# ksil/LFPSQP.jl

Hardware: AMD Instinct MI355X
Metric: projected-CG iters/sec at n=1e7, m=128 fp64 (higher is better)
Workload: dtype f64

## Files before the change

lfpsqp.jl_amd/csrc/context.hip:

```cpp
#include <dlfcn.h>
#include <stdarg.h>
#include <stdio.h>
#include <stdlib.h>
#include <ctype.h>
#include <string.h>

#include <algorithm>

#include "internal.h"

namespace lfpsqp {

int set_err(lfpsqp_ctx* ctx, int code, const char* fmt, ...) {
    char buf[1024];
    va_list ap;
    va_start(ap, fmt);
    vsnprintf(buf, sizeof(buf), fmt, ap);
    va_end(ap);
    if (ctx) ctx->err = buf;
    else fprintf(stderr, "lfpsqp: %s\n", buf);
    return code;
}

int ensure_part(lfpsqp_ctx* ctx, size_t doubles) {
// ... 228 lines not shown
}

__global__ __launch_bounds__(lfpsqp::kThreads) void view_copy_kernel(const double* __restrict__ A, const double* __restrict__ rs, const double* __restrict__ u,
                                                                     const double* __restrict__ w, double* __restrict__ D, int64_t ld, int64_t n, int m) {
    const int64_t i = ((int64_t)blockIdx.x * lfpsqp::kThreads + threadIdx.x) * 2;
    if (i >= n) return;
    const double2 s = rs ? lfpsqp::ld2(rs + i) : make_double2(1.0, 1.0);
    const double2 uu = u ? lfpsqp::ld2(u + i) : make_double2(0.0, 0.0);
    const bool v1 = i + 1 < n;
    const int j0 = blockIdx.y * 16, j1 = (j0 + 16 < m) ? j0 + 16 : m;
#pragma unroll 4
    for (int j = j0; j < j1; ++j) {
        const double2 c = lfpsqp::ld2(A + (int64_t)j * ld + i);
        const double wj = u ? w[j] : 0.0;
        const double2 o = make_double2(fma(uu.x, wj, s.x * c.x), fma(uu.y, wj, s.y * c.y));
        if (v1) lfpsqp::st2(D + (int64_t)j * ld + i, o);
        else D[(int64_t)j * ld + i] = o.x;
    }
}

extern "C" {

int lfpsqp_ctx_create(int device, lfpsqp_ctx** out) {
    if (!out) return LFPSQP_ERR_ARG;
    *out = nullptr;
    int ndev = 0;
    if (hipGetDeviceCount(&ndev) != hipSuccess || ndev <= 0) return set_err(nullptr, LFPSQP_ERR_HIP, "no HIP device visible");
    if (device < 0 || device >= ndev) return set_err(nullptr, LFPSQP_ERR_ARG, "device %d out of range (%d visible)", device, ndev);
    lfpsqp_ctx* ctx = new lfpsqp_ctx();
    ctx->device = device;
    if (hipSetDevice(device) != hipSuccess) { delete ctx; return set_err(nullptr, LFPSQP_ERR_HIP, "hipSetDevice(%d) failed", device); }
    hipDeviceProp_t prop;
    if (hipGetDeviceProperties(&prop, device) == hipSuccess) {
        ctx->devname = std::string(prop.name) + " (" + prop.gcnArchName + ")";
        ctx->num_cu = prop.multiProcessorCount;
        ctx->real_gpu = strncmp(prop.gcnArchName, "gfx", 3) == 0;
    }
    bool ok = hipStreamCreate(&ctx->stream) == hipSuccess;
    ok = ok && hipMalloc((void**)&ctx->scal, 64 * sizeof(double)) == hipSuccess;
    ok = ok && hipMalloc((void**)&ctx->istat, 128 * sizeof(int64_t)) == hipSuccess;
    ok = ok && hipHostMalloc((void**)&ctx->h_scal, 4 * 64 * sizeof(double)) == hipSuccess;
    ok = ok && hipHostMalloc((void**)&ctx->h_istat, 4 * 16 * sizeof(int64_t)) == hipSuccess;
    for (int i = 0; ok && i < 4; ++i) ok = hipEventCreate(&ctx->ev_slot[i]) == hipSuccess;
    ok = ok && hipEventCreate(&ctx->ev_t0) == hipSuccess && hipEventCreate(&ctx->ev_t1) == hipSuccess;
    if (ok) ok = hipMemset(ctx->scal, 0, 64 * sizeof(double)) == hipSuccess && hipMemset(ctx->istat, 0, 128 * sizeof(int64_t)) == hipSuccess;
    if (!ok) { delete ctx; return set_err(nullptr, LFPSQP_ERR_HIP, "context resource allocation failed"); }
    if (const char* e = getenv("LFPSQP_ONEPASS")) ctx->tune_onepass = atoi(e);
    if (const char* e = getenv("LFPSQP_SPGRAM")) ctx->tune_spgram = atoi(e) < 0 ? -1 : 0;
    if (const char* e = getenv("LFPSQP_VEC_BLOCKS")) ctx->tune_vec_blocks = atoi(e) > 0 ? atoi(e) : 0;
    if (const char* e = getenv("LFPSQP_NRB_MFMA")) ctx->tune_nrb_mfma = atoi(e) > 0 ? 1 : (atoi(e) < 0 ? -1 : 0);
    if (const char* e = getenv("LFPSQP_GPING")) ctx->tune_gping = atoi(e) == 1 ? 1 : 0;
    if (const char* e = getenv("LFPSQP_NRB_WG_CAP")) ctx->batch_wg_cap = atoi(e) > 0 ? atoi(e) : 0;
    if (const char* e = getenv("LFPSQP_STAGE_ROUNDS")) ctx->stage_cap = atoi(e) > 0 ? atoi(e) : 0;
    *out = ctx;
    return 0;
}

int lfpsqp_ctx_destroy(lfpsqp_ctx* ctx) {
    if (!ctx) return 0;
    (void)hipSetDevice(ctx->device);
    (void)hipStreamSynchronize(ctx->stream);
    if (ctx->comm.kind == Comm::RCCL && ctx->comm.nccl_comm && ctx->comm.ncclCommDestroy) ctx->comm.ncclCommDestroy(ctx->comm.nccl_comm);
    for (int r = 0; r < kP2PMaxRanks; ++r)
        if (ctx->comm.p2p_peer[r] && ctx->comm.p2p_peer[r] != ctx->comm.p2p_mine) (void)hipIpcCloseMemHandle(ctx->comm.p2p_peer[r]);
    if (ctx->comm.p2p_mine) (void)hipFree(ctx->comm.p2p_mine);
    if (ctx->comm.p2p_err) (void)hipHostFree(ctx->comm.p2p_err);
    if (ctx->prof_init)
        for (int s = 0; s < kProfSlots; ++s)
            for (int e = 0; e < kProfEvents; ++e)
                for (int k = 0; k < 2; ++k) (void)hipEventDestroy(ctx->prof_ev[s][e][k]);
    for (int i = 0; i < 4; ++i) if (ctx->ev_slot[i]) (void)hipEventDestroy(ctx->ev_slot[i]);
    if (ctx->ev_t0) (void)hipEventDestroy(ctx->ev_t0);
    if (ctx->ev_t1) (void)hipEventDestroy(ctx->ev_t1);
    if (ctx->part) (void)hipFree(ctx->part);
    if (ctx->small) (void)hipFree(ctx->small);
    if (ctx->d_m) (void)hipFree(ctx->d_m);
    if (ctx->d_qw) (void)hipFree(ctx->d_qw);
    if (ctx->d_zeros) (void)hipFree(ctx->d_zeros);
    if (ctx->d_nvec) (void)hipFree(ctx->d_nvec);
    if (ctx->d_tri) (void)hipFree(ctx->d_tri);
    if (ctx->d_view) (void)hipFree(ctx->d_view);
    if (ctx->h_m) (void)hipHostFree(ctx->h_m);
    if (ctx->scal) (void)hipFree(ctx->scal);
    if (ctx->istat) (void)hipFree(ctx->istat);
    if (ctx->h_scal) (void)hipHostFree(ctx->h_scal);
    if (ctx->h_istat) (void)hipHostFree(ctx->h_istat);
    if (ctx->stream) (void)hipStreamDestroy(ctx->stream);
    delete ctx;
    return 0;
}

int lfpsqp_ctx_sync(lfpsqp_ctx* ctx) {
    LF_ARG(ctx, ctx != nullptr);
    LF_HIP(ctx, hipStreamSynchronize(ctx->stream));
    return 0;
}

const char* lfpsqp_last_error(const lfpsqp_ctx* ctx) { return ctx ? ctx->err.c_str() : "null context"; }

int lfpsqp_device_name(const lfpsqp_ctx* ctx, char* buf, int64_t buflen) {
    if (!ctx || !buf || buflen <= 0) return LFPSQP_ERR_ARG;
    snprintf(buf, (size_t)buflen, "%s", ctx->devname.c_str());
    return 0;
}

int lfpsqp_device_uuid(const lfpsqp_ctx* ctx, char* buf, int64_t buflen) {
// ... 588 lines not shown
```

lfpsqp.jl_amd/csrc/internal.h:

```cpp
#pragma once
#include <hip/hip_runtime.h>
#include <stdint.h>

#include <string>
#include <vector>

#include "../../include/lfpsqp_hip.h"
#include "kernels.h"

struct lfpsqp_slab {
    void* p = nullptr;
    int refs = 0;
};
struct lfpsqp_vec {
    double* p = nullptr;
    int64_t n = 0;
    int64_t cap = 0;
    lfpsqp_slab* slab = nullptr;
};

constexpr int64_t kLdSkewDefault = 16;

struct lfpsqp_mat {
    double* p = nullptr;
// ... 42 lines not shown

    double* part = nullptr;
    size_t part_cap = 0;
    double* small = nullptr;
    size_t small_cap = 0;
    double* d_m = nullptr;
    double* h_m = nullptr;
    size_t m_cap = 0;
    std::vector<double> warm_V;
    int warm_m = 0;
    double* d_view = nullptr;
    double* d_nvec = nullptr;
    size_t nvec_cap = 0;
    double* d_tri = nullptr;
    size_t tri_cap = 0;
    double* d_zeros = nullptr;
    double* d_qw = nullptr;
    size_t qw_cap = 0;
    double* scal = nullptr;
    int64_t* istat = nullptr;
    double* h_scal = nullptr;
    int64_t* h_istat = nullptr;
    hipEvent_t ev_slot[4] = {nullptr, nullptr, nullptr, nullptr};
    hipEvent_t ev_t0 = nullptr, ev_t1 = nullptr;

    int tune_ks = 0;
    bool tune_nt = true;
    int ks_for(int64_t n) const { return tune_ks ? tune_ks : (n >= 4000000 ? 4 : 2); }
    int tune_onepass = 0;
    int tune_spgram = 0;
    int tune_vec_blocks = 0;
    int tune_nrb_mfma = -1;
    int tune_gping = 0;

    bool real_gpu = false;
    int place_tries = 3;
    int64_t place_min_bytes = (int64_t)1 << 30;
    double place_last_ms[64] = {0};
    int place_last_n = 0, place_last_pick = 0;

    struct ProjcgResume {
        bool valid = false;
        const double *x = nullptr, *g = nullptr, *d = nullptr, *Z = nullptr;
        int m = 0;
        int64_t nv = 0, iters = 0;
        bool gcur_is_rp = false;
        const double *dg = nullptr, *b = nullptr;
        double a0 = 0.0;
        int64_t n_global = 0;
        uint64_t epoch = 0;
    } pcg_resume;
    int batch_wg_cap = 0;
    int stage_cap = 0;
    uint64_t launch_epoch = 0;

    bool profiling = false;
    hipEvent_t prof_ev[lfpsqp::kProfSlots][lfpsqp::kProfEvents][2];
    int prof_used[lfpsqp::kProfSlots] = {0};
    int64_t prof_seq[lfpsqp::kProfSlots] = {0};
    bool prof_live[lfpsqp::kProfSlots] = {false};
    int64_t prof_count[lfpsqp::kProfSlots] = {0};
    double prof_ms[lfpsqp::kProfSlots] = {0};
    bool prof_init = false;
};

namespace lfpsqp {

int set_err(lfpsqp_ctx* ctx, int code, const char* fmt, ...);
int ensure_part(lfpsqp_ctx* ctx, size_t doubles);
int ensure_small(lfpsqp_ctx* ctx, size_t doubles);
int ensure_mvec(lfpsqp_ctx* ctx, size_t doubles);
int ensure_nvec(lfpsqp_ctx* ctx, size_t doubles);
int ensure_view(lfpsqp_ctx* ctx);
constexpr int kViewTau = 8;
constexpr int kViewScratch = kViewTau + 4 * 1024 + 64;
int allreduce_dev(lfpsqp_ctx* ctx, double* buf, int64_t count, int op = 0);

void prof_begin(lfpsqp_ctx* ctx, int s);
void prof_end(lfpsqp_ctx* ctx, int s);
void prof_collect(lfpsqp_ctx* ctx);

inline int64_t round_up(int64_t a, int64_t b) { return (a + b - 1) / b * b; }
inline int64_t ntiles_of(int64_t n, int ks) { return (n + (int64_t)kSlabRows * ks - 1) / ((int64_t)kSlabRows * ks); }

#define LF_HIP(ctx, expr)                                                                              \
    do {                                                                                               \
        hipError_t e__ = (expr);                                                                       \
        if (e__ != hipSuccess)                                                                         \
            return lfpsqp::set_err((ctx), LFPSQP_ERR_HIP, "%s failed: %s (%s:%d)", #expr,              \
                                   hipGetErrorString(e__), __FILE__, __LINE__);                        \
    } while (0)

#define LF_TRY(expr)               \
    do {                           \
        int rc__ = (expr);         \
        if (rc__ != 0) return rc__; \
    } while (0)

#define LF_ARG(ctx, cond)                                                                               \
    do {                                                                                                \
        if (!(cond)) return lfpsqp::set_err((ctx), LFPSQP_ERR_ARG, "invalid argument: %s (%s:%d)", #cond, \
                                            __FILE__, __LINE__);                                        \
    } while (0)

#define LF_LAUNCH_CHECK(ctx) LF_HIP(ctx, hipGetLastError())

// ... 355 lines not shown
```

lfpsqp.jl_amd/csrc/projcg.hip:

```cpp
#include <math.h>
#include <stdlib.h>

#include <algorithm>
#include <vector>

#include "internal.h"
#include "sparse.h"
#include "sphess.h"

namespace lfpsqp {

enum { S_DAD = 0, S_RG = 1, S_ALPHA = 2, S_RPGP = 3, S_GPGP = 4, S_BETA = 5, S_NR = 6, S_TOL = 7, S_DD = 8, S_ALPHA_PREV = 9 };
enum { I_STATUS = 0, I_ITER = 1, I_MAXIT = 2 };
enum { ST_RUNNING = 0, ST_CONVERGED = 1, ST_RG_BREAK = 2, ST_NEGCURV = 3, ST_MAXIT = 4 };

struct AOpD {
    double a0;
    const double* dg;
    __device__ __forceinline__ double2 apply(int64_t i, double2 d) const {
        if (dg) {
            const double2 q = ld2(dg + i);
            return make_double2((a0 + q.x) * d.x, (a0 + q.y) * d.y);
        }
        return make_double2(a0 * d.x, a0 * d.y);
    }
};

struct AOpV {
    const double* Av;
    __device__ __forceinline__ double2 apply(int64_t i, double2) const { return ld2(Av + i); }
};

struct AOpLR {
    double a0;
    const double* dg;
    const double* V;
    int64_t ldv;
    int k;
    const double *sigma, *vtv;
    __device__ __forceinline__ double2 apply(int64_t i, double2 d) const {
        double2 o = dg ? make_double2((a0 + dg[i]) * d.x, (a0 + dg[i + 1]) * d.y) : make_double2(a0 * d.x, a0 * d.y);
        for (int j = 0; j < k; ++j) {
            const double c = ld_scal(sigma + j) * ld_scal(vtv + j);
            const double2 v = ld2(V + (int64_t)j * ldv + i);
            o.x = fma(v.x, c, o.x);
            o.y = fma(v.y, c, o.y);
        }
        return o;
    }
};

template <int B>
struct BandD {
    static_assert(B >= 1 && B <= 4, "bandwidth 1 .. 4");
    double a0;
    const double* dg;
    const double* off;
    int64_t ldo;
    int64_t n;
    int64_t nc;
    __device__ __forceinline__ const double* col(int k) const { return off + (int64_t)(k - 1) * ldo; }
};
template <int B>
struct TriMulF {
    BandD<B> A;
    const double* v;
// ... 719 lines not shown
                red[0] += (h == 2) ? rr * ar : gp * ((h == 0) ? rr : ((h == 1) ? gp : w.ad));
                if (h == 0) red[1] += w.dx * w.ad;
            }
            v[0] = valid ? gp : 0.0;
            v[1] = valid ? ar : 0.0;
        } else {
            const double acc = accv[0];
            const double ady = w.ay * w.dy;
            const double rx = INIT ? w.gx : fma(u.alpha, w.ad, w.gx);
            const double ry = INIT ? w.gy : fma(u.alpha, ady, w.gy);
            const double ww = w.Dx * rx + w.Dy * ry;
            const double ux = rx - w.Dx * ww, uy = ry - w.Dy * ww;
            const double gx = rx - fma(w.sx, acc, w.Dx * ww);
            const double gy = ry - fma(w.sy, acc, w.Dy * ww);
            const double aux = fma(w.ax, ux, w.q), auy = w.ay * uy;
            if (valid && owner) {
                if (slot) { slot[0] = gx; slot[sstride] = gy; }
                else { put(gout, o, gx); put(gout + k.hs, o, gy); }
                if (INIT) { put(d, o, -gx); put(d + k.hs, o, -gy); }
            }
            if (valid && lead) {
                const double px = (h == 2) ? ux : gx, py = (h == 2) ? uy : gy;
                const double fx = (h == 0) ? rx : ((h == 1) ? gx : ((h == 2) ? aux : w.ad));
                const double fy = (h == 0) ? ry : ((h == 1) ? gy : ((h == 2) ? auy : ady));
                red[0] += fx * px + fy * py;
                if (h == 0) red[1] += w.dx * w.ad + w.dy * ady;
            }
            v[0] = valid ? (w.sx * gx + w.sy * gy) : 0.0;
            v[1] = valid ? (w.sx * aux + w.sy * auy) : 0.0;
        }
    }
};

struct PcgPostF {
    const double* T;
    double* t3;
    double* Utr;
    double* scal;
    int64_t* istat;
    int m, init;
    HostMirror hm;
    const double* W = nullptr;
    const double* Traw = nullptr;
    double* Tw = nullptr;
    double* uA = nullptr;
    int wm = 0;
    int pre = 0;
    int k = 0;
    const double* UtV = nullptr;
    const double* sigma = nullptr;
    double* vdraw = nullptr;
    double* vdc = nullptr;
    const double* triM = nullptr;
    __device__ __forceinline__ int nsums() const { return k > 0 ? 5 + kLRMax : 5; }
};
template <int NY>
__device__ __forceinline__ void small_wdot(const double* W, size_t ld, size_t sk, int rows, int cols, const double* const (&x)[NY], const double* xs,
                                           double (&y)[NY], double* scratch ) {
    int rp = 32;
    while (rp < rows) rp <<= 1;
    const int groups = (int)blockDim.x / rp > 0 ? (int)blockDim.x / rp : 1;
    const int j = threadIdx.x % rp, g = threadIdx.x / rp;
    double acc[NY];
#pragma unroll
    for (int q = 0; q < NY; ++q) acc[q] = 0.0;
    if (j < rows && g < groups)
        for (int k = g; k < cols; k += groups) {
            const double w = W[(size_t)j * ld + (size_t)k * sk];
#pragma unroll
            for (int q = 0; q < NY; ++q) acc[q] = fma(w, xs ? xs[k] : ld_scal(x[q] + k), acc[q]);
        }
#pragma unroll
    for (int q = 0; q < NY; ++q) scratch[q * blockDim.x + threadIdx.x] = acc[q];
    __syncthreads();
#pragma unroll
    for (int q = 0; q < NY; ++q) {
        double sum = 0.0;
        if (g == 0 && j < rows)
            for (int gg = 0; gg < groups; ++gg) sum += scratch[q * blockDim.x + gg * rp + j];
        y[q] = sum;
    }
    __syncthreads();
}

__global__ __launch_bounds__(1024) void pcg_post_kernel(PcgPostF u) {
    if (u.init == 2) {
        if (threadIdx.x == 0) u.istat[I_STATUS] = ST_RUNNING;
        __syncthreads();
    } else if (ld_stat(u.istat + I_STATUS) != ST_RUNNING) return;
    __shared__ double sh[2];
    __shared__ int go;
    __shared__ double s_utr[kOnepassMaxCols];
    __shared__ double s_part[2 * 1024];
    if (u.W && u.init != 2 && !u.pre) {
        const double* const xin[2] = {u.Traw, u.Traw + u.wm};
        double yo[2];
        small_wdot<2>(u.W, (size_t)u.wm, 1, u.m, u.wm, xin, nullptr, yo, s_part);
        if ((int)threadIdx.x < u.m) {
            int rp = 32;
            while (rp < u.m) rp <<= 1;
            if ((int)threadIdx.x / rp == 0) { u.Tw[threadIdx.x] = yo[0]; u.Tw[u.m + threadIdx.x] = yo[1]; }
        }
        if ((int)threadIdx.x < u.nsums()) u.Tw[2 * u.m + threadIdx.x] = ld_scal(u.Traw + 2 * u.wm + threadIdx.x);
        __threadfence();
        __syncthreads();
    }
    __shared__ double s_mu[kOnepassMaxCols];
    __shared__ double s_tri[2];
    if (u.triM) {
        for (int j = threadIdx.x; j < u.m; j += blockDim.x) s_utr[j] = ld_scal(u.Utr + j);
        __syncthreads();
        double c1 = 0.0, c2 = 0.0;
        for (int j = threadIdx.x; j < u.m; j += blockDim.x) {
            double a = 0.0;
            for (int l = 0; l < u.m; ++l) a = fma(u.triM[(size_t)l * u.m + j], s_utr[l], a);
            s_mu[j] = a;
            c1 = fma(ld_scal(u.T + u.m + j), s_utr[j], c1);
            c2 = fma(a, s_utr[j], c2);
        }
        s_part[threadIdx.x] = c1;
        s_part[1024 + threadIdx.x] = c2;
        __syncthreads();
        for (int w = (int)blockDim.x >> 1; w > 0; w >>= 1) {
            if ((int)threadIdx.x < w) {
                s_part[threadIdx.x] += s_part[threadIdx.x + w];
                s_part[1024 + threadIdx.x] += s_part[1024 + threadIdx.x + w];
            }
            __syncthreads();
        }
        if (threadIdx.x == 0) { s_tri[0] = s_part[0]; s_tri[1] = s_part[1024]; }
        __syncthreads();
    }
    if (threadIdx.x == 0) {
        const double* S = u.T + 2 * u.m;
        const double rpgp = ld_scal(S), gpgp = ld_scal(S + 1), gAd = ld_scal(S + 3), dAd = ld_scal(S + 4);
        double gAg = ld_scal(S + 2);
        if (u.triM) gAg = (gAg - 2.0 * s_tri[0]) + s_tri[1];
        for (int j = 0; j < u.k; ++j) {
            const double vg = ld_scal(S + 5 + j);
            gAg = fma(ld_scal(u.sigma + j) * vg, vg, gAg);
        }
        double beta = 0.0, dAd_next = gAg;
        int64_t it = 0;
        int64_t st = ST_RUNNING;
        double nr = INFINITY;
        if (u.init == 1) {
            u.scal[S_RG] = gpgp;
            if (ld_stat(u.istat + I_MAXIT) <= 0) st = ST_MAXIT;
            u.hm.publish(st, 0, INFINITY);
        } else if (u.init == 2) {
            beta = ld_scal(u.scal + S_BETA);
            nr = ld_scal(u.scal + S_NR);
            it = ld_stat(u.istat + I_ITER);
            if (it >= ld_stat(u.istat + I_MAXIT)) st = ST_MAXIT;
            u.hm.publish(st, it, nr);
            dAd_next = fma(beta * beta, dAd, fma(-2.0 * beta, gAd, gAg));
        } else {
            beta = rpgp / ld_scal(u.scal + S_RG);
            u.scal[S_BETA] = beta;
            u.scal[S_RG] = gpgp;
            nr = sqrt(gpgp);
            u.scal[S_NR] = nr;
            it = ld_stat(u.istat + I_ITER);
            if (nr < ld_scal(u.scal + S_TOL)) st = ST_CONVERGED;
            else if (it >= ld_stat(u.istat + I_MAXIT)) st = ST_MAXIT;
            u.hm.publish(st, it, nr);
            dAd_next = fma(beta * beta, dAd, fma(-2.0 * beta, gAd, gAg));
        }
        if (st == ST_RUNNING) {
            u.istat[I_ITER] = it + 1;
            u.scal[S_DAD] = dAd_next;
            if (dAd_next <= 0.0) st = ST_NEGCURV;
            else if (gpgp <= 0.0) st = ST_RG_BREAK;
            else {
                u.scal[S_ALPHA_PREV] = (u.init == 2) ? 0.0 : ld_scal(u.scal + S_ALPHA);
                u.scal[S_ALPHA] = gpgp / dAd_next;
            }
            if (st != ST_RUNNING) u.hm.publish(st, it + 1, nr);
        }
        if (st != ST_RUNNING) u.istat[I_STATUS] = st;
        go = (st == ST_RUNNING);
        sh[0] = gpgp / dAd_next;
        sh[1] = beta;
        if (go)
            for (int j = 0; j < u.k; ++j) {
                const double vg = ld_scal(S + 5 + j);
                const double vd = (u.init == 1) ? -vg : fma(beta, u.vdraw[j], -vg);
                u.vdraw[j] = vd;
                u.vdc[j] = ld_scal(u.sigma + j) * vd;
            }
    }
    __syncthreads();
    if (!go) return;
    const double alpha = sh[0], beta = sh[1];
    for (int j = threadIdx.x; j < u.m; j += blockDim.x) {
        const double t1 = ld_scal(u.T + j);
        double t2 = ld_scal(u.T + u.m + j);
        if (u.triM) t2 -= s_mu[j];
        for (int l = 0; l < u.k; ++l)
            t2 = fma(u.UtV[(size_t)l * u.m + j], ld_scal(u.sigma + l) * ld_scal(u.T + 2 * u.m + 5 + l), t2);
        const double t3 = (u.init == 1) ? -t2 : fma(beta, u.t3[j], -t2);
        u.t3[j] = t3;
        const double ut = fma(alpha, t3, t1);
        u.Utr[j] = ut;
        if (u.W) s_utr[j] = ut;
    }
    if (u.W) {
        __syncthreads();
        const double* const xin[1] = {nullptr};
        double yo[1];
        small_wdot<1>(u.W, 1, (size_t)u.wm, u.wm, u.m, xin, s_utr, yo, s_part);
        int rp = 32;
        while (rp < u.wm) rp <<= 1;
        if ((int)threadIdx.x < u.wm && (int)threadIdx.x / rp == 0) u.uA[threadIdx.x] = yo[0];
    }
}
#ifndef LFPSQP_K1_NT
#define LFPSQP_K1_NT 1
#endif
struct PcgDirG {
    double* d;
    const double* g;
    double* x;
    const double* scal;
    const int64_t* istat;
    int force;
    __device__ __forceinline__ bool skip() const { return !force && ld_stat(istat + I_STATUS) != ST_RUNNING; }
    __device__ __forceinline__ void apply(int64_t i, bool v0, bool v1, double*) const {
        double2 dd = ld2(d + i);
        if (!force) {
            const double alpha = ld_scal(scal + S_ALPHA_PREV);
            double2 xx = ld2(x + i);
            xx = make_double2(fma(alpha, dd.x, xx.x), fma(alpha, dd.y, xx.y));
            if (v1) { if (LFPSQP_K1_NT >= 1) st2_stream(x + i, xx); else st2(x + i, xx); }
            else if (v0) x[i] = xx.x;
        }
        const double beta = ld_scal(scal + S_BETA);
        const double2 gg = ld2(g + i);
        dd = make_double2(beta * dd.x - gg.x, beta * dd.y - gg.y);
        if (v1) { if (LFPSQP_K1_NT == 1) st2_stream(d + i, dd); else st2(d + i, dd); }
        else if (v0) d[i] = dd.x;
    }
};

template <class AOP>
struct ResidualV {
    const double* x;
    const double* b;
    double* out;
    AOP A;
    double sgn;
    __device__ __forceinline__ bool skip() const { return false; }
    __device__ __forceinline__ double2 load(int64_t r, bool v0, bool v1) const {
        const double2 xx = ld2(x + r), bb = ld2(b + r);
        const double2 ax = A.apply(r, xx);
        const double2 rr = make_double2(sgn * (ax.x - bb.x), sgn * (ax.y - bb.y));
        if (out) {
            if (v1) st2(out + r, rr);
            else if (v0) out[r] = rr.x;
        }
        return make_double2(v0 ? rr.x : 0.0, v1 ? rr.y : 0.0);
    }
};
struct InitState {
    double* scal;
    int64_t* istat;
    double tol;
    int64_t maxit;
    __device__ __forceinline__ bool skip() const { return false; }
    __device__ __forceinline__ void run(double*) const {
        for (int k = 0; k < 16; ++k) scal[k] = 0.0;
        scal[S_TOL] = tol;
        scal[S_NR] = INFINITY;
        istat[I_STATUS] = ST_RUNNING;
        istat[I_ITER] = 0;
        istat[I_MAXIT] = maxit;
    }
};
struct FlushXF {
    double* x;
    const double* d;
    const double* scal;
    __device__ __forceinline__ bool skip() const { return false; }
    __device__ __forceinline__ void apply(int64_t i, bool v0, bool v1, double*) const {
        const double alpha = ld_scal(scal + S_ALPHA);
        const double2 dd = ld2(d + i);
        double2 xx = ld2(x + i);
        xx = make_double2(fma(alpha, dd.x, xx.x), fma(alpha, dd.y, xx.y));
        if (v1) st2(x + i, xx);
        else if (v0) x[i] = xx.x;
    }
};
struct SumSqF {
    const double* x;
    __device__ __forceinline__ bool skip() const { return false; }
    __device__ __forceinline__ void apply(int64_t i, bool v0, bool v1, double* red) const {
        const double2 a = ld2(x + i);
        double s = 0.0;
        if (v0) s = a.x * a.x;
        if (v1) s = fma(a.y, a.y, s);
        red[0] += s;
    }
};
struct NormalizeIntoF {
    double* x;
    const double* d;
    const double* dd;
    __device__ __forceinline__ bool skip() const { return false; }
    __device__ __forceinline__ void apply(int64_t i, bool v0, bool v1, double*) const {
        const double nrm = sqrt(ld_scal(dd));
        const double2 a = ld2(d + i);
        const double2 o = make_double2(a.x / nrm, a.y / nrm);
        if (v1) st2(x + i, o);
        else if (v0) x[i] = o.x;
    }
};

template <class AOP>
struct PcgStepVS {
    PcgStepV<AOP> p;
    StackD k;
    __device__ __forceinline__ bool skip() const { return p.skip(); }
    __device__ __forceinline__ double2 load(int64_t r, bool v0, bool v1) const {
        const double2 rx = p.load(r, v0, v1);
        const double2 ry = p.load(r + k.hs, v0, v1);
        const double2 ax = ld2(k.sx + r), ay = ld2(k.sy + r);
        return make_double2(ax.x * rx.x + ay.x * ry.x, ax.y * rx.y + ay.y * ry.y);
    }
};
template <class AOP>
struct ResidualVS {
    ResidualV<AOP> p;
    StackD k;
    double* wout;
    __device__ __forceinline__ bool skip() const { return false; }
    __device__ __forceinline__ double2 load(int64_t r, bool v0, bool v1) const {
// ... 562 lines not shown

    const bool kPing = ctx->tune_gping == 1;
    double* gbuf[2] = {g, (fused && kPing && !cop) ? rp : g};
    int gcur = 0;
    auto prepare_neighbours = [&](auto STc, auto INc, const double* src, const double* dsrc, double* ad, double* q) -> int {
        constexpr bool ST = decltype(STc)::value, INIT = decltype(INc)::value;
        if (cop->kind == CoupledOp::BAND)
            return with_band(cop->K, [&](auto Bc) -> int {
                constexpr int B = decltype(Bc)::value;
                const BandD<B> Ab = cop->template band<B>(N, N);
                if constexpr (ST) return run_vec<TriPrepSF<B, INIT>, 0, NoPost>(ctx, N, TriPrepSF<B, INIT>{Ab, hs, sk.Dx, sk.Dy, src, dsrc, ad, q, scal, istat}, 0u, nullptr, NoPost());
                else return run_vec<TriPrepF<B, INIT>, 0, NoPost>(ctx, N, TriPrepF<B, INIT>{Ab, src, dsrc, ad, q, scal, istat}, 0u, nullptr, NoPost());
            });
        return with_gathers(*cop, N, N, [&](auto Ab) -> int {
            using D = decltype(Ab);
            if constexpr (ST) {
                double* ux = ctx->d_tri;
                LF_TRY((run_vec<DiagsPrepSF<D, INIT>, 0, NoPost>(ctx, N, DiagsPrepSF<D, INIT>{Ab, hs, sk.Dx, sk.Dy, src, dsrc, ad, ux, scal, istat}, 0u, nullptr, NoPost())));
                return run_vec<DiagsGatherF<D>, 0, NoPost>(ctx, N, DiagsGatherF<D>{Ab, ux, nullptr, q, scal, istat}, 0u, nullptr, NoPost());
            } else {
                if constexpr (!INIT) LF_TRY((run_vec<DiagsMulF<D>, 0, NoPost>(ctx, N, DiagsMulF<D>{Ab, dsrc, ad, istat}, 0u, nullptr, NoPost())));
                return run_vec<DiagsGatherF<D>, 0, NoPost>(ctx, N, DiagsGatherF<D>{Ab, src, ad, q, scal, istat}, 0u, nullptr, NoPost());
            }
        });
    };
    auto launch_fused = [&](int init) -> int {
        const int slot = init ? -1 : 3;
        const double* gin = gbuf[gcur];
        double* gout = init ? gbuf[0] : gbuf[gcur ^ 1];
        const double* tin = DF ? uDF : Utr;
        double* Tout = DF ? Traw : T12;
        auto fuse_lr = [&](auto INc) -> int {
            constexpr bool INIT = decltype(INc)::value;
            return run_onepass<PcgFuseLR<INIT>, 2, 5 + kLRMax>(ctx, Z, mc, mc, N, tin, PcgFuseLR<INIT>{rp, gin, gout, d, Ad, scal, istat, LRop->V->p, LRop->V->ld, kLR, lrVdc}, Tout, slot);
        };
        if (cop) LF_TRY(with_stacked_init(stacked, init != 0, [&](auto STc, auto INc) -> int {
            constexpr bool ST = decltype(STc)::value, INIT = decltype(INc)::value;
            const double* src = INIT ? rp : gin;
            const double* dsrc = INIT ? nullptr : d;
            double* ad = INIT ? nullptr : Av->p;
            double* q = INIT ? Av->p : rp;
            LF_TRY(prepare_neighbours(STc, INc, src, dsrc, ad, q));
            return run_onepass<PcgFuseTri<ST, INIT>, 2, 5>(ctx, Z, mc, mc, N, tin, PcgFuseTri<ST, INIT>{rp, gin, gout, d, ad, q, Ad, scal, istat, sk}, Tout, slot);
        }));
        else if (kLR > 0) LF_TRY(init ? fuse_lr(std::true_type{}) : fuse_lr(std::false_type{}));
        else LF_TRY(with_stacked_init(stacked, init != 0, [&](auto STc, auto INc) -> int {
            constexpr bool ST = decltype(STc)::value, INIT = decltype(INc)::value;
            return run_onepass<PcgFuseE<ST, INIT>, 2, 5>(ctx, Z, mc, mc, N, tin, PcgFuseE<ST, INIT>{rp, gin, gout, d, Ad, scal, istat, sk}, Tout, slot);
        }));
        if (!init) gcur ^= 1;
        PcgPostF pf{T12, t3, Utr, scal, istat, m, init, hm, dWf, Traw, T12, uDF, DF ? mc : 0};
        if (kLR > 0) { pf.k = kLR; pf.UtV = lrUtV; pf.sigma = lrSig; pf.vdraw = lrVdraw; pf.vdc = lrVdc; }
        pf.triM = dTriM;
        hipLaunchKernelGGL(pcg_post_kernel, dim3(1), dim3(DF ? 1024 : 256), 0, ctx->stream, pf);
        LF_LAUNCH_CHECK(ctx);
        return 0;
    };

    const bool resume = (flags & LFPSQP_PROJCG_RESUME) != 0;
    int64_t it_base = 0;
    if (resume) {
        if (!fused || !rs.valid || rs.x != x->p || rs.g != g || rs.d != d || rs.Z != Z->p || rs.m != m || rs.nv != nv || rs.dg != Ad.dg ||
            rs.a0 != Ad.a0 || rs.b != b->p || rs.n_global != n_global || rs.epoch != ctx->launch_epoch)
            return set_err(ctx, LFPSQP_ERR_UNSUPPORTED, "LFPSQP_PROJCG_RESUME: no resumable projcg state for these arguments "
                           "(needs the one-pass iteration, a previous call with the same x, A, U, b, work that stopped at its iteration limit, and no library call that queued device work in between)");
        it_base = rs.iters;
        gcur = (rs.gcur_is_rp && gbuf[1] == rp) ? 1 : 0;
        if (rs.gcur_is_rp != (gcur == 1)) return set_err(ctx, LFPSQP_ERR_UNSUPPORTED, "LFPSQP_PROJCG_RESUME: the buffer scheme changed between the calls");
        maxit_eff = (it_base + maxit < n_global + m_ref) ? it_base + maxit : n_global + m_ref;
        hstat[1] = it_base;
        const int64_t lim = maxit_eff;
        LF_HIP(ctx, hipMemcpyAsync(istat + I_MAXIT, &lim, sizeof(int64_t), hipMemcpyHostToDevice, ctx->stream));
        LF_HIP(ctx, hipStreamSynchronize(ctx->stream));
        hipLaunchKernelGGL(pcg_post_kernel, dim3(1), dim3(DF ? 1024 : 256), 0, ctx->stream, PcgPostF{T12, t3, Utr, scal, istat, m, 2, hm, dWf, Traw, T12, uDF, DF ? mc : 0});
        LF_LAUNCH_CHECK(ctx);
    }
    ctx->pcg_resume.valid = false;
    if (!resume) {
        hipLaunchKernelGGL((post_kernel<InitState>), dim3(1), dim3(1), 0, ctx->stream, scal, InitState{scal, istat, tol, maxit_eff});
        LF_LAUNCH_CHECK(ctx);

        if (c && m > 0) {
            if (!DF) LF_TRY(lfpsqp_gemv_n(ctx, Z, m, 1.0, c, 0.0, x));
        } else {
            LF_TRY(lfpsqp_vec_fill(ctx, x, 0.0));
        }
        if (kLR > 0) {
            for (int j = 0; j < kLRMax; ++j) ctx->h_m[j] = (j < kLR) ? (LRop->sigma ? LRop->sigma[j] : 1.0) : 0.0;
            LF_HIP(ctx, hipMemcpyAsync(lrSig, ctx->h_m, sizeof(double) * kLRMax, hipMemcpyHostToDevice, ctx->stream));
            LF_HIP(ctx, hipStreamSynchronize(ctx->stream));
            LF_HIP(ctx, hipMemsetAsync(lrVdraw, 0, sizeof(double) * 3 * kLRMax, ctx->stream));
            for (int l = 0; l < kLR; ++l) {
                const SpPlainV col{LRop->V->p + (int64_t)l * LRop->V->ld};
                if (DF) LF_TRY(df_gemv_t(col, lrUtV + (size_t)l * m, nullptr));
                else LF_TRY(run_gemv_t(ctx, Z, m, N, col, lrUtV + (size_t)l * m));
            }
        }
        if (flags & LFPSQP_PROJCG_START_PROJECTED) {
            if (!(DF && fused && !c && kLR == 0) || work->Utr->n < (int64_t)mc + 2 * m + 5)
                return set_err(ctx, LFPSQP_ERR_UNSUPPORTED, "LFPSQP_PROJCG_START_PROJECTED: basis in factored form over a dense generator, c == NULL, work->Utr of >= A.m + 2 ncols + 5 entries");
            LF_HIP(ctx, hipMemcpyAsync(T12, Utr + mc, sizeof(double) * (2 * (size_t)m + 5), hipMemcpyDeviceToDevice, ctx->stream));
            PcgPostF pf{T12, t3, Utr, scal, istat, m, 1, hm, dWf, Traw, T12, uDF, mc};
            pf.pre = 1;
            hipLaunchKernelGGL(pcg_post_kernel, dim3(1), dim3(1024), 0, ctx->stream, pf);
            LF_LAUNCH_CHECK(ctx);
        } else if (flags & LFPSQP_PROJCG_START_GIVEN) {
            if (!(DF && fused && !c))
                return set_err(ctx, LFPSQP_ERR_UNSUPPORTED, "LFPSQP_PROJCG_START_GIVEN: basis in factored form over a dense generator, c == NULL");
            LF_TRY(factored_w_times_t(ctx, dWf, mc, m, Utr, uDF));
        } else {
            LF_TRY(launch_residual(1.0, rp, Utr));
        }
        if (flags & LFPSQP_PROJCG_START_PROJECTED) {  }
        else if (fused) LF_TRY(launch_fused(1));
        else LF_TRY(launch_k3(1));
    }

    int64_t it = 0;
    bool done = false;
    const int gcur_start = gcur;
    const int64_t it_end = maxit_eff - it_base;
    while (!done && it < it_end) {
        if (fused) {
            if (it > 0 || resume) LF_TRY((run_vec<PcgDirG, 0, NoPost>(ctx, nv, PcgDirG{d, gbuf[gcur], x->p, scal, istat, 0}, 0u, nullptr, NoPost(), 0)));
            LF_TRY(launch_fused(0));
        } else if (callback) {
            if (it > 0) LF_TRY((run_vec<PcgDirX, 0, NoPost>(ctx, nv, PcgDirX{d, g, x->p, scal, istat}, 0u, nullptr, NoPost(), 0)));
            LF_TRY(apply_op(work->d));
            LF_TRY((run_vec<DotPairF, 1, PcgPost1>(ctx, nv, DotPairF{d, Av->p, istat}, 0u, scal + S_DAD, PcgPost1{scal, istat, hm})));
            LF_TRY(launch_k2());
            LF_TRY(launch_k3(0));
        } else {
            LF_TRY((run_vec<PcgDirF, 1, PcgPost1>(ctx, nv, PcgDirF{d, g, x->p, Ad, scal, istat, it == 0 ? 1 : 0}, 0u, scal + S_DAD,
                                                  PcgPost1{scal, istat, hm}, 0)));
            LF_TRY(launch_k2());
            LF_TRY(launch_k3(0));
        }
        LF_HIP(ctx, hipEventRecord(ctx->ev_slot[it & 3], ctx->stream));
        if (it >= 2) {
            LF_HIP(ctx, hipEventSynchronize(ctx->ev_slot[(it - 2) & 3]));
            if (hstat[kRingOff + ((it_base + it - 1) % kRing)] != ST_RUNNING) done = true;
        }
        ++it;
    }
    LF_HIP(ctx, hipStreamSynchronize(ctx->stream));
    const int64_t status = hstat[0];
    *iters = hstat[1];
    *nr = *(volatile double*)ctx->h_scal;
    if (fused) {
        const int64_t executed = ((status == ST_CONVERGED || status == ST_MAXIT) ? *iters : *iters - 1) - it_base;
        gcur = (gbuf[1] != gbuf[0]) ? (int)((gcur_start + (executed > 0 ? executed : 0)) & 1) : 0;
    }

    if ((status == ST_CONVERGED || status == ST_MAXIT || (fused && status == ST_RG_BREAK && *iters > 1)) && *iters > it_base)
        LF_TRY((run_vec<FlushXF, 0, NoPost>(ctx, nv, FlushXF{x->p, d, scal}, 0u, nullptr, NoPost())));
    if (fused && status == ST_MAXIT && *iters > 0 && kLR == 0 && !cop)
        ctx->pcg_resume = lfpsqp_ctx::ProjcgResume{true, x->p, g, d, Z->p, m, nv, *iters, gcur == 1, Ad.dg, b->p, Ad.a0, n_global, ctx->launch_epoch};
    if (status == ST_NEGCURV) {
        if (fused && *iters > 1)
            LF_TRY((run_vec<PcgDirG, 0, NoPost>(ctx, nv, PcgDirG{d, gbuf[gcur], x->p, scal, istat, 1}, 0u, nullptr, NoPost())));
        LF_TRY((run_vec<SumSqF, 1, NoPost>(ctx, nv, SumSqF{d}, 0u, scal + S_DD, NoPost())));
        LF_TRY((run_vec<NormalizeIntoF, 0, NoPost>(ctx, nv, NormalizeIntoF{x->p, d, scal + S_DD}, 0u, nullptr, NoPost())));
        if (lambda) LF_TRY(lfpsqp_vec_fill(ctx, lambda, NAN));
        *nr = INFINITY;
    } else if (flags & LFPSQP_PROJCG_WANT_LAMBDA) {
        if (stacked) LF_TRY(launch_residual(-1.0, nullptr, lambda->p + N));
        else if (m > 0) LF_TRY(launch_residual(-1.0, nullptr, lambda->p));
    }
    if (ctx->profiling) {
        LF_HIP(ctx, hipStreamSynchronize(ctx->stream));
        prof_collect(ctx);
    }
    return 0;
}

int lfpsqp::placement_probe(lfpsqp_ctx* ctx, const lfpsqp_mat* M, int ncols, double* g, double* d, double* a, int reps, double* ms) {
    *ms = -1.0;
    if (!M || M->n <= 0 || ncols < 4 || ncols > M->m || onepass_cw(ctx, ncols, M->ld, M->n) == 0) return 0;
    LF_TRY(ensure_mvec(ctx, (size_t)3 * ncols + 24));
    double* T12 = ctx->d_m;
    double* Utr = ctx->d_m + round_up(2 * ncols + 5, 2);
    LF_HIP(ctx, hipMemsetAsync(ctx->d_m, 0, sizeof(double) * ((size_t)3 * ncols + 24), ctx->stream));
    hipLaunchKernelGGL((post_kernel<InitState>), dim3(1), dim3(1), 0, ctx->stream, ctx->scal, InitState{ctx->scal, ctx->istat, 0.0, (int64_t)1 << 40});
    LF_LAUNCH_CHECK(ctx);
    const StackD sk{0, nullptr, nullptr, nullptr, nullptr};
    const Comm::Kind saved = ctx->comm.kind;
    ctx->comm.kind = Comm::NONE;
    int rc = 0;
    for (int k = 0; k < reps + 1 && rc == 0; ++k) {
        if (k == 1) rc = hipEventRecord(ctx->ev_t0, ctx->stream) == hipSuccess ? 0 : LFPSQP_ERR_HIP;
        if (rc == 0) rc = with_stacked_init(false, false, [&](auto STc, auto INc) -> int {
            constexpr bool ST = decltype(STc)::value, INIT = decltype(INc)::value;
            return run_onepass<PcgFuseE<ST, INIT>, 2, 5>(ctx, M, ncols, ncols, M->n, Utr, PcgFuseE<ST, INIT>{g, g, g, d, AOpD{0.0, a}, ctx->scal, ctx->istat, sk}, T12, -1);
        });
    }
    ctx->comm.kind = saved;
    LF_TRY(rc);
    LF_HIP(ctx, hipEventRecord(ctx->ev_t1, ctx->stream));
    LF_HIP(ctx, hipEventSynchronize(ctx->ev_t1));
    float t = 0.f;
    LF_HIP(ctx, hipEventElapsedTime(&t, ctx->ev_t0, ctx->ev_t1));
    *ms = (double)t / reps;
    return 0;
}

extern "C" int lfpsqp_projcg(lfpsqp_ctx* ctx, lfpsqp_vec* x, lfpsqp_vec* lambda, const lfpsqp_diag_op* A, const lfpsqp_basis* U,
                             const lfpsqp_vec* b, const lfpsqp_vec* c, double tol, int64_t maxit, int64_t n_global, int flags,
                             const lfpsqp_projcg_work* work, int64_t* iters, double* nr) {
    LF_RANGE("lfpsqp_projcg");
    LF_ARG(ctx, ctx && A);
    return projcg_impl(ctx, x, lambda, PcgOperator{PcgOperator::DIAGONAL, *A}, U, b, c, tol, maxit, n_global, flags, work, iters, nr);
}

// ... 134 lines not shown
```

Before: 593.3.

## Defer x updates to every other projected-CG iteration

The fused direction-update kernel now updates x only on alternate iterations. It folds the previous step and the current step (alpha_prev*d_prev + alpha*d_new) into a single read-modify-write of x, and skips x entirely on the other iterations. The aim is to roughly halve x memory traffic in the bandwidth-bound vector pass. A device flag records whether an x update is still owed, so the final flush is skipped when nothing is pending. An env knob restores per-iteration updates. This adds parity-dependent control state and a risk of getting x wrong on resume or early-exit paths.

Result: no change. 609.4, median of 6 (+2.7%).

```diff
diff --git a/lfpsqp.jl_amd/csrc/context.hip b/lfpsqp.jl_amd/csrc/context.hip
--- a/lfpsqp.jl_amd/csrc/context.hip
+++ b/lfpsqp.jl_amd/csrc/context.hip
@@ -304,6 +304,7 @@
     if (const char* e = getenv("LFPSQP_GPING")) ctx->tune_gping = atoi(e) == 1 ? 1 : 0;
     if (const char* e = getenv("LFPSQP_NRB_WG_CAP")) ctx->batch_wg_cap = atoi(e) > 0 ? atoi(e) : 0;
     if (const char* e = getenv("LFPSQP_STAGE_ROUNDS")) ctx->stage_cap = atoi(e) > 0 ? atoi(e) : 0;
+    if (const char* e = getenv("LFPSQP_X_EVERY")) ctx->x_every = atoi(e) == 1 ? 1 : 2;
     *out = ctx;
     return 0;
 }
diff --git a/lfpsqp.jl_amd/csrc/internal.h b/lfpsqp.jl_amd/csrc/internal.h
--- a/lfpsqp.jl_amd/csrc/internal.h
+++ b/lfpsqp.jl_amd/csrc/internal.h
@@ -118,6 +118,7 @@
     } pcg_resume;
     int batch_wg_cap = 0;
     int stage_cap = 0;
+    int x_every = 2;
     uint64_t launch_epoch = 0;
 
     bool profiling = false;
diff --git a/lfpsqp.jl_amd/csrc/projcg.hip b/lfpsqp.jl_amd/csrc/projcg.hip
--- a/lfpsqp.jl_amd/csrc/projcg.hip
+++ b/lfpsqp.jl_amd/csrc/projcg.hip
@@ -11,7 +11,7 @@
 namespace lfpsqp {
 
 enum { S_DAD = 0, S_RG = 1, S_ALPHA = 2, S_RPGP = 3, S_GPGP = 4, S_BETA = 5, S_NR = 6, S_TOL = 7, S_DD = 8, S_ALPHA_PREV = 9 };
-enum { I_STATUS = 0, I_ITER = 1, I_MAXIT = 2 };
+enum { I_STATUS = 0, I_ITER = 1, I_MAXIT = 2, I_XOWED = 3 };
 enum { ST_RUNNING = 0, ST_CONVERGED = 1, ST_RG_BREAK = 2, ST_NEGCURV = 3, ST_MAXIT = 4 };
 
 struct AOpD {
@@ -837,6 +837,7 @@
     double* vdraw = nullptr;
     double* vdc = nullptr;
     const double* triM = nullptr;
+    int xe = 2;
     __device__ __forceinline__ int nsums() const { return k > 0 ? 5 + kLRMax : 5; }
 };
 template <int NY>
@@ -937,6 +938,7 @@
             beta = ld_scal(u.scal + S_BETA);
             nr = ld_scal(u.scal + S_NR);
             it = ld_stat(u.istat + I_ITER);
+            u.istat[I_XOWED] = 0;
             if (it >= ld_stat(u.istat + I_MAXIT)) st = ST_MAXIT;
             u.hm.publish(st, it, nr);
             dAd_next = fma(beta * beta, dAd, fma(-2.0 * beta, gAd, gAg));
@@ -960,6 +962,7 @@
             else {
                 u.scal[S_ALPHA_PREV] = (u.init == 2) ? 0.0 : ld_scal(u.scal + S_ALPHA);
                 u.scal[S_ALPHA] = gpgp / dAd_next;
+                u.istat[I_XOWED] = (u.xe == 1 || ((it + 1) & 1)) ? 1 : 0;
             }
             if (st != ST_RUNNING) u.hm.publish(st, it + 1, nr);
         }
@@ -1010,19 +1013,28 @@
     const double* scal;
     const int64_t* istat;
     int force;
+    int xe;
     __device__ __forceinline__ bool skip() const { return !force && ld_stat(istat + I_STATUS) != ST_RUNNING; }
     __device__ __forceinline__ void apply(int64_t i, bool v0, bool v1, double*) const {
         double2 dd = ld2(d + i);
-        if (!force) {
+        const int steps = force ? 0 : (xe == 1 ? 1 : ((ld_stat(istat + I_ITER) & 1) ? 0 : 2));
+        double2 xx = make_double2(0.0, 0.0);
+        if (steps) {
             const double alpha = ld_scal(scal + S_ALPHA_PREV);
-            double2 xx = ld2(x + i);
+            xx = ld2(x + i);
             xx = make_double2(fma(alpha, dd.x, xx.x), fma(alpha, dd.y, xx.y));
-            if (v1) { if (LFPSQP_K1_NT >= 1) st2_stream(x + i, xx); else st2(x + i, xx); }
-            else if (v0) x[i] = xx.x;
         }
         const double beta = ld_scal(scal + S_BETA);
         const double2 gg = ld2(g + i);
         dd = make_double2(beta * dd.x - gg.x, beta * dd.y - gg.y);
+        if (steps == 2) {
+            const double alpha = ld_scal(scal + S_ALPHA);
+            xx = make_double2(fma(alpha, dd.x, xx.x), fma(alpha, dd.y, xx.y));
+        }
+        if (steps) {
+            if (v1) { if (LFPSQP_K1_NT >= 1) st2_stream(x + i, xx); else st2(x + i, xx); }
+            else if (v0) x[i] = xx.x;
+        }
         if (v1) { if (LFPSQP_K1_NT == 1) st2_stream(d + i, dd); else st2(d + i, dd); }
         else if (v0) d[i] = dd.x;
     }
@@ -1066,7 +1078,8 @@
     double* x;
     const double* d;
     const double* scal;
-    __device__ __forceinline__ bool skip() const { return false; }
+    const int64_t* owed;
+    __device__ __forceinline__ bool skip() const { return owed != nullptr && ld_stat(owed) == 0; }
     __device__ __forceinline__ void apply(int64_t i, bool v0, bool v1, double*) const {
         const double alpha = ld_scal(scal + S_ALPHA);
         const double2 dd = ld2(d + i);
@@ -1735,6 +1748,7 @@
         PcgPostF pf{T12, t3, Utr, scal, istat, m, init, hm, dWf, Traw, T12, uDF, DF ? mc : 0};
         if (kLR > 0) { pf.k = kLR; pf.UtV = lrUtV; pf.sigma = lrSig; pf.vdraw = lrVdraw; pf.vdc = lrVdc; }
         pf.triM = dTriM;
+        pf.xe = ctx->x_every;
         hipLaunchKernelGGL(pcg_post_kernel, dim3(1), dim3(DF ? 1024 : 256), 0, ctx->stream, pf);
         LF_LAUNCH_CHECK(ctx);
         return 0;
@@ -1755,7 +1769,9 @@
         const int64_t lim = maxit_eff;
         LF_HIP(ctx, hipMemcpyAsync(istat + I_MAXIT, &lim, sizeof(int64_t), hipMemcpyHostToDevice, ctx->stream));
         LF_HIP(ctx, hipStreamSynchronize(ctx->stream));
-        hipLaunchKernelGGL(pcg_post_kernel, dim3(1), dim3(DF ? 1024 : 256), 0, ctx->stream, PcgPostF{T12, t3, Utr, scal, istat, m, 2, hm, dWf, Traw, T12, uDF, DF ? mc : 0});
+        PcgPostF pf{T12, t3, Utr, scal, istat, m, 2, hm, dWf, Traw, T12, uDF, DF ? mc : 0};
+        pf.xe = ctx->x_every;
+        hipLaunchKernelGGL(pcg_post_kernel, dim3(1), dim3(DF ? 1024 : 256), 0, ctx->stream, pf);
         LF_LAUNCH_CHECK(ctx);
     }
     ctx->pcg_resume.valid = false;
@@ -1785,6 +1801,7 @@
             LF_HIP(ctx, hipMemcpyAsync(T12, Utr + mc, sizeof(double) * (2 * (size_t)m + 5), hipMemcpyDeviceToDevice, ctx->stream));
             PcgPostF pf{T12, t3, Utr, scal, istat, m, 1, hm, dWf, Traw, T12, uDF, mc};
             pf.pre = 1;
+            pf.xe = ctx->x_every;
             hipLaunchKernelGGL(pcg_post_kernel, dim3(1), dim3(1024), 0, ctx->stream, pf);
             LF_LAUNCH_CHECK(ctx);
         } else if (flags & LFPSQP_PROJCG_START_GIVEN) {
@@ -1805,7 +1822,10 @@
     const int64_t it_end = maxit_eff - it_base;
     while (!done && it < it_end) {
         if (fused) {
-            if (it > 0 || resume) LF_TRY((run_vec<PcgDirG, 0, NoPost>(ctx, nv, PcgDirG{d, gbuf[gcur], x->p, scal, istat, 0}, 0u, nullptr, NoPost(), 0)));
+            if (it > 0 || resume) {
+                const bool visits_x = ctx->x_every == 1 || ((it_base + it + 1) & 1) == 0;
+                LF_TRY((run_vec<PcgDirG, 0, NoPost>(ctx, nv, PcgDirG{d, gbuf[gcur], x->p, scal, istat, 0, ctx->x_every}, 0u, nullptr, NoPost(), visits_x ? 0 : -1)));
+            }
             LF_TRY(launch_fused(0));
         } else if (callback) {
             if (it > 0) LF_TRY((run_vec<PcgDirX, 0, NoPost>(ctx, nv, PcgDirX{d, g, x->p, scal, istat}, 0u, nullptr, NoPost(), 0)));
@@ -1836,12 +1856,12 @@
     }
 
     if ((status == ST_CONVERGED || status == ST_MAXIT || (fused && status == ST_RG_BREAK && *iters > 1)) && *iters > it_base)
-        LF_TRY((run_vec<FlushXF, 0, NoPost>(ctx, nv, FlushXF{x->p, d, scal}, 0u, nullptr, NoPost())));
+        LF_TRY((run_vec<FlushXF, 0, NoPost>(ctx, nv, FlushXF{x->p, d, scal, fused ? istat + I_XOWED : nullptr}, 0u, nullptr, NoPost())));
     if (fused && status == ST_MAXIT && *iters > 0 && kLR == 0 && !cop)
         ctx->pcg_resume = lfpsqp_ctx::ProjcgResume{true, x->p, g, d, Z->p, m, nv, *iters, gcur == 1, Ad.dg, b->p, Ad.a0, n_global, ctx->launch_epoch};
     if (status == ST_NEGCURV) {
         if (fused && *iters > 1)
-            LF_TRY((run_vec<PcgDirG, 0, NoPost>(ctx, nv, PcgDirG{d, gbuf[gcur], x->p, scal, istat, 1}, 0u, nullptr, NoPost())));
+            LF_TRY((run_vec<PcgDirG, 0, NoPost>(ctx, nv, PcgDirG{d, gbuf[gcur], x->p, scal, istat, 1, ctx->x_every}, 0u, nullptr, NoPost())));
         LF_TRY((run_vec<SumSqF, 1, NoPost>(ctx, nv, SumSqF{d}, 0u, scal + S_DD, NoPost())));
         LF_TRY((run_vec<NormalizeIntoF, 0, NoPost>(ctx, nv, NormalizeIntoF{x->p, d, scal + S_DD}, 0u, nullptr, NoPost())));
         if (lambda) LF_TRY(lfpsqp_vec_fill(ctx, lambda, NAN));
```
